# tkeskita/smoothMesh

Measured on AMD Instinct MI355X. Metric: mesh-points smoothed/sec/node (100 iters) + achieved HBM GB/s vs roofline, higher is better.
Workload: dtype f64

## Files before the change

### smoothmesh_amd/csrc/kernels_tiled.hpp

```cpp
#pragma once
#include "kernels.hpp"
#include "tile_meta.hpp"

#ifndef SMGPU_STAGGER
#define SMGPU_STAGGER 0
#endif
__device__ __forceinline__ void staggerFirstRound(int bid, int resident) {
#if SMGPU_STAGGER
    if (bid < resident) {
        const unsigned slot = __builtin_amdgcn_s_getreg((3 << 11) | (0 << 6) | 4) & 15u;
        for (unsigned k = 0; k < slot; ++k) __builtin_amdgcn_s_sleep(SMGPU_STAGGER);
    }
#else
    (void)bid; (void)resident;
#endif
}
#ifndef SMGPU_ABLATE
#define SMGPU_ABLATE 0
#endif
namespace smgpu {

constexpr unsigned kPad = 0xFFFFu;

struct GeomTileView {
// ... 447 lines not shown
    if (tm.nPts > 2 * T)
        stageRecords<T, 2, kGP>(s.ptsCur, g.tpIds + tm.tpOff + 2 * T, tm.nPts - 2 * T, L.px + kGP * 2 * T, L.py + kGP * 2 * T, L.pz + kGP * 2 * T, tid);
}
template <int T, bool ORG>
__device__ __forceinline__ void geomFaces(const State& s, const GeomTileView& g, const GeomLds& L, const GeomTileMeta& tm, const GeomRows& r, int tid,
                                          int wantAvg, int writeFaces) {
    const unsigned tflags = (unsigned)tm.flags;
    const int nf = tm.nFaces;
#pragma unroll
    for (int u = 0; u < 2; ++u) {
        const int i = u * T + tid;
        if (i < nf) geomFace<ORG>(s, g, L, tm, i, tflags, wantAvg, writeFaces, r.preFaces, r.fq[u]);
    }
    for (int i = 2 * T + tid; i < nf; i += T) geomFace<ORG>(s, g, L, tm, i, tflags, wantAvg, writeFaces);
}

template <int T, bool ORG>
__device__ __forceinline__ void geomTileBody(const TileLaunch& tl, const MeshView& m, const State& s, const GeomTileView& g, int wantAvg, int writeFaces,
                                             int deferN, int deferIter, double* deferLocal, double* deferHist, int bid, bool coh = false) {
    const int tile = launchedTile(tl, bid);
    if (tile < 0) return;
    const GeomTileMeta tm = loadGeomMeta(tl.meta, tile);
    const int stopped = stopWord(tl);
    scalarBatch(tm.tpOff, tm.nPts, tm.tfOff, tm.nFaces, tm.fvBase, tm.fvWidth, tm.cellBeg, tm.nCells, tm.cfBase, tm.cfWidth, tm.flags, stopped,
                g.tpIds, g.faceVerts, g.cellOrder, g.cellFaces, s.ptsCur, deferN);
    staggerFirstRound(bid, 256 * 4);
    if (deferN > 0 && bid == 0) { if (stopped) return; finishPartials<T>(s, deferN, deferIter, -1.0, deferLocal, deferHist); __syncthreads(); }
    extern __shared__ double lds[];
    const int tid = threadIdx.x;
    const GeomLds L = geomLds(lds, tm);
    int id[2];
    geomLoadIds<T>(g, tm, tid, id);
    const GeomRows r = geomLoadRows<T, ORG>(g, tm, tid);
    V3 v[2];
    geomLoadPoints(s, id, v);
    geomStorePoints<T>(s, g, tm, L, id, v, tid);
    if (stopped) return;
    prologuePrioDown<1>();
    __syncthreads();
    if (SMGPU_ABLATE & 32) { if (tid < tm.nCells) stv(s.cellCtr, ((const_int_ptr)g.cellOrder)[tm.cellBeg + tid], v3(L.px[tid], 0.0, 0.0)); return; }
    geomFaces<T, ORG>(s, g, L, tm, r, tid, wantAvg, writeFaces);
    __syncthreads();
    if (SMGPU_ABLATE & 64) return;
    geomCell<T, ORG>(s, g, L, tm, tid, (unsigned)tm.flags, r.cin, coh);
}
template <int T, bool ORG>
__global__ void __launch_bounds__(T, (SMGPU_GEOM_WAVES * T) / 256) k_geom_tile(TileLaunch tl, MeshView m, State s, GeomTileView g, int wantAvg, int writeFaces,
                                                  int deferN, int deferIter, double* deferLocal, double* deferHist) {
    prologuePrioUp<1>();
    geomTileBody<T, ORG>(tl, m, s, g, wantAvg, writeFaces, deferN, deferIter, deferLocal, deferHist, (int)blockIdx.x);
}

struct SmoothLds { double *cx, *cy, *cz, *nx, *ny, *nz; };
__device__ __forceinline__ SmoothLds smoothLds(double* lds, const SmoothTileMeta& tm) {
    SmoothLds L;
    L.cx = lds;                 L.cy = L.cx + tm.nCells;  L.cz = L.cy + tm.nCells;
    L.nx = L.cz + tm.nCells;    L.ny = L.nx + tm.nNbrs;   L.nz = L.ny + tm.nNbrs;
    return L;
}
struct Top3 {
    double l1 = 0, l2 = 0, l3 = 0;
    unsigned w1 = 0xFFFFFFFFu, w2 = 0xFFFFFFFFu, w3 = 0xFFFFFFFFu;
    __device__ __forceinline__ void offer(double len, int j, unsigned e, bool take) {
        const unsigned w = ((unsigned)j << 16) | e;
        const bool b1 = take && (w1 == 0xFFFFFFFFu || len < l1);
        const bool b2 = take && !b1 && (w2 == 0xFFFFFFFFu || len < l2);
        const bool b3 = take && !b1 && !b2 && (w3 == 0xFFFFFFFFu || len < l3);
        const bool b12 = b1 || b2;
        l3 = b12 ? l2 : (b3 ? len : l3);  w3 = b12 ? w2 : (b3 ? w : w3);
        l2 = b1 ? l1 : (b2 ? len : l2);   w2 = b1 ? w1 : (b2 ? w : w2);
        l1 = b1 ? len : l1;               w1 = b1 ? w : w1;
    }
    __device__ __forceinline__ bool has2() const { return w2 != 0xFFFFFFFFu; }
    __device__ __forceinline__ bool has3() const { return w3 != 0xFFFFFFFFu; }
    __device__ __forceinline__ int k1() const { return (int)(w1 >> 16); }
    __device__ __forceinline__ int k2() const { return (int)(w2 >> 16); }
};
struct SmoothRow {
    bool mine; int p, selfL, wn4, wc4, slot;
    int peer, dst0, ndst;
    unsigned fl;
    const ushort4 *ppRow, *pcRow;
    ushort4 pp0, pp1, pc0, pc1;
    ushort4 pe0, pe1;
};
template <int T>
__device__ __forceinline__ unsigned pairBits(const SmoothTileView& g, const SmoothTileMeta& tm, const SmoothRow& R, int tid, int k) {
    if (k < 8) {
        const ushort4 q = (k & 4) ? R.pe1 : R.pe0;
        const unsigned lo = (k & 1) ? q.y : q.x, hi = (k & 1) ? q.w : q.z;
        return (k & 2) ? hi : lo;
    }
    const uint16_t* pe = g.pairEll + tm.ppBase;
    return pe[((size_t)(k >> 2) * T + tid) * 4 + (k & 3)];
}
struct SlotTabs { const int* slot; const int* peer; const int* dst0; const int* ndst; };
template <int T, bool COHC = false, int SLOTS = 1>
__device__ __forceinline__ SmoothRow smoothStage(const MeshView& m, const State& s, const SmoothTileView& g, const SmoothTileMeta& tm,
                                                 const SmoothLds& L, int tid, const SlotTabs& tb = SlotTabs{nullptr, nullptr, nullptr, nullptr}) {
    scalarBatch(tm.ptBeg, tm.nPts, tm.tcOff, tm.nCells, tm.tnOff, tm.nNbrs, tm.pcBase, tm.pcWidth, tm.ppBase, tm.ppWidth,
                g.tcIds, g.tnIds, g.ptOrder, g.selfLoc, g.ppEll, g.pcEll, g.pairEll, g.usePairShare, s.cellCtr, s.ptsCur, m.pflags);
    if (SLOTS == 1) scalarBatch(s.sharedSlot);
    if (SLOTS == 2) scalarBatch(tb.slot, tb.peer, tb.dst0, tb.ndst);
    SmoothRow r;
    r.peer = -1; r.dst0 = -1; r.ndst = 0;
    r.mine = tid < tm.nPts;
    r.wn4 = tm.ppWidth >> 2; r.wc4 = tm.pcWidth >> 2;
    const int lane = r.mine ? tid : 0;
    r.ppRow = reinterpret_cast<const ushort4*>(g.ppEll + tm.ppBase) + tid;
    r.pcRow = reinterpret_cast<const ushort4*>(g.pcEll + tm.pcBase) + tid;
    const bool fast = tm.nCells <= 2 * T && tm.nNbrs <= 3 * T && r.wn4 > 0 && r.wc4 > 0;
    const ushort4 padq = make_ushort4(0xFFFF, 0xFFFF, 0xFFFF, 0xFFFF);
    if (fast) {
        const int* ic = g.tcIds + tm.tcOff;
        const int* in = g.tnIds + tm.tnOff;
        int a[2], b[3];
#pragma unroll
        for (int u = 0; u < 2; ++u) { const int i = u * T + tid; a[u] = (i < tm.nCells) ? ic[i] : -1; }
#pragma unroll
        for (int u = 0; u < 3; ++u) { const int i = u * T + tid; b[u] = (i < tm.nNbrs) ? in[i] : -1; }
        const int pi = tm.ptBeg + lane;
        const int p = g.ptOrder[pi];
        const int selfL = g.selfLoc[pi];
        const ushort4* ppl = reinterpret_cast<const ushort4*>(g.ppEll + tm.ppBase) + lane;
        const ushort4* pcl = reinterpret_cast<const ushort4*>(g.pcEll + tm.pcBase) + lane;
        const ushort4 pp0 = ppl[0], pp1 = ppl[r.wn4 > 1 ? T : 0], pc0 = pcl[0], pc1 = pcl[r.wc4 > 1 ? T : 0];
        const ushort4* pel = reinterpret_cast<const ushort4*>((g.usePairShare ? g.pairEll : g.ppEll) + tm.ppBase) + lane;
        r.pe0 = pel[0]; r.pe1 = pel[r.wn4 > 1 ? T : 0];
        int slot = -1, peer = -1, dst0 = -1, ndst = 0;
        if (SLOTS == 2) { slot = tb.slot[pi]; if (tb.peer) { peer = tb.peer[pi]; dst0 = tb.dst0[pi]; ndst = tb.ndst[pi]; } }
        V3 va[2], vb[3];
#pragma unroll
        for (int u = 0; u < 2; ++u) va[u] = (a[u] >= 0) ? (COHC ? ldvCoh(s.cellCtr, a[u]) : ldv(s.cellCtr, a[u])) : v3(0, 0, 0);
#pragma unroll
        for (int u = 0; u < 3; ++u) vb[u] = (b[u] >= 0) ? ldv(s.ptsCur, b[u]) : v3(0, 0, 0);
        const unsigned fl = m.pflags[p];
        if (SLOTS == 1) slot = s.sharedSlot ? s.sharedSlot[p] : -1;
#pragma unroll
        for (int u = 0; u < 2; ++u) { const int i = u * T + tid; if (a[u] >= 0) { L.cx[i] = va[u].x; L.cy[i] = va[u].y; L.cz[i] = va[u].z; } }
#pragma unroll
        for (int u = 0; u < 3; ++u) { const int i = u * T + tid; if (b[u] >= 0) { L.nx[i] = vb[u].x; L.ny[i] = vb[u].y; L.nz[i] = vb[u].z; } }
        r.p = r.mine ? p : 0; r.selfL = r.mine ? selfL : 0;
        r.fl = fl; r.slot = r.mine ? slot : -1; r.peer = r.mine ? peer : -1; r.dst0 = dst0; r.ndst = r.mine ? ndst : 0;
        r.pp0 = r.mine ? pp0 : padq; r.pp1 = (r.mine && r.wn4 > 1) ? pp1 : padq;
        r.pc0 = r.mine ? pc0 : padq; r.pc1 = (r.mine && r.wc4 > 1) ? pc1 : padq;
        return r;
    }
    r.p = 0; r.selfL = 0; r.fl = 0; r.slot = -1;
    r.pp0 = padq; r.pp1 = padq; r.pc0 = padq; r.pc1 = padq; r.pe0 = padq; r.pe1 = padq;
    if (r.mine) {
        if (g.usePairShare) {
            const ushort4* peRow = reinterpret_cast<const ushort4*>(g.pairEll + tm.ppBase) + tid;
            if (r.wn4 > 0) r.pe0 = peRow[0];
            if (r.wn4 > 1) r.pe1 = peRow[T];
        }
        const int pi = tm.ptBeg + tid;
        r.p = g.ptOrder[pi];
        r.selfL = g.selfLoc[pi];
        if (r.wn4 > 0) r.pp0 = r.ppRow[0];
        if (r.wn4 > 1) r.pp1 = r.ppRow[T];
        if (r.wc4 > 0) r.pc0 = r.pcRow[0];
        if (r.wc4 > 1) r.pc1 = r.pcRow[T];
        r.fl = m.pflags[r.p];
        if (SLOTS == 1) r.slot = s.sharedSlot ? s.sharedSlot[r.p] : -1;
        if (SLOTS == 2) { r.slot = tb.slot[pi]; if (tb.peer) { r.peer = tb.peer[pi]; r.dst0 = tb.dst0[pi]; r.ndst = tb.ndst[pi]; } }
    }
    if (COHC) stageRecordsCoh<T>(s.cellCtr, g.tcIds + tm.tcOff, tm.nCells, L.cx, L.cy, L.cz, tid);
    else stageRecords<T, 2>(s.cellCtr, g.tcIds + tm.tcOff, tm.nCells, L.cx, L.cy, L.cz, tid);
    stageRecords<T, 3>(s.ptsCur, g.tnIds + tm.tnOff, tm.nNbrs, L.nx, L.ny, L.nz, tid);
    return r;
}

template <bool FINAL, int T, int MODE = 0>
__device__ __forceinline__ void smoothPoint(const MeshView& m, const State& s, const Prm& prm, const SmoothTileView& g, const SmoothLds& L,
                                            const SmoothRow& R, const SmoothTileMeta& tm, int tid, double& dist, int& fcount, bool spTile = false) {
    const double *cx = L.cx, *cy = L.cy, *cz = L.cz, *nx = L.nx, *ny = L.ny, *nz = L.nz;
    const bool mine = R.mine;
    const int p = R.p, selfL = R.selfL, wn4 = R.wn4, wc4 = R.wc4;
    const ushort4 *ppRow = R.ppRow, *pcRow = R.pcRow;
    const ushort4 pp0 = R.pp0, pp1 = R.pp1, pc0 = R.pc0, pc1 = R.pc1;
    if ((SMGPU_ABLATE & 16) && !spTile) { if (mine) stv(FINAL ? s.ptsNext : s.prop, p, ldsv(nx, ny, nz, selfL)); return; }
    if (mine && !(MODE == 2 && !spTile && R.slot >= 0)) {
        const unsigned fl = R.fl;
        const bool internal = fl & PF_INTERNAL;
        const V3 cur = ldsv(nx, ny, nz, selfL);
        V3 sum = v3(0, 0, 0), r1, r2, r3;
        double m1 = 0.0, m2 = 0.0, m3 = 0.0;
        int count = 0, hc = 0;
        double shortestCur = SMGPU_GREAT;
        const int slot = (MODE == 1 || (MODE == 2 && !spTile)) ? -1 : R.slot;
        if (slot >= 0) {
            {
                const double* r = s.combA + (size_t)slot * SMGPU_HALO_A_DOUBLES;
                double w[SMGPU_HALO_A_DOUBLES];
#pragma unroll
                for (int q = 0; q < SMGPU_HALO_A_DOUBLES; ++q) w[q] = (MODE == 2 && R.peer < 0) ? ldCoh(r + q) : r[q];
                sum = v3(w[0], w[1], w[2]);
                r1 = v3(w[3], w[4], w[5]); r2 = v3(w[6], w[7], w[8]); r3 = v3(w[9], w[10], w[11]);
                const long long pk = __double_as_longlong(w[12]);
                count = (int)(pk & 0xffffffffll);
                hc = (int)(pk >> 32);
            }
            m1 = mag(r1); m2 = mag(r2); m3 = mag(r3);
            SMGPU_ELL_FOREACH_PRE(pp0, pp1, ppRow, wn4, T, {
                (void)j;
                const double len = mag(cur - ldsv(nx, ny, nz, e & 0x7fff));
                if (len < shortestCur) shortestCur = len;
            })
        } else {
            if (internal || prm.bndOn) {
                if (!(SMGPU_ABLATE & 8))
                SMGPU_ELL_FOREACH_PRE(pc0, pc1, pcRow, wc4, T, {
                    sum = sum + ldsv(cx, cy, cz, (SMGPU_ABLATE & 2) ? 0 : e);
                    count = j + 1;
                })
            }
            Top3 t3;
            SMGPU_ELL_FOREACH_PRE(pp0, pp1, ppRow, wn4, T, {
                const V3 dv_ = cur - ldsv(nx, ny, nz, (SMGPU_ABLATE & 2) ? 0 : (e & 0x7fff));
                const double len = (SMGPU_ABLATE & 1) ? magSqr(dv_) : mag(dv_);
                if (len < shortestCur) shortestCur = len;
                t3.offer(len, j, e, internal || !(e & 0x8000));
            })
            if (!t3.has2()) { s.acc->err = 1; r1 = r2 = r3 = v3(0, 0, 0); }
            else {
                r1 = ldsv(nx, ny, nz, t3.w1 & 0x7fff) - cur;
                r2 = ldsv(nx, ny, nz, t3.w2 & 0x7fff) - cur;
                r3 = !t3.has3() ? v3(SMGPU_GREAT, SMGPU_GREAT, SMGPU_GREAT) : ldsv(nx, ny, nz, t3.w3 & 0x7fff) - cur;
                m1 = t3.l1; m2 = t3.l2; m3 = !t3.has3() ? mag(r3) : t3.l3;
                if (g.usePairShare) {
                    hc = (pairBits<T>(g, tm, R, tid, t3.k1()) >> t3.k2()) & 1;
                } else {
                    const int nb = m.ppOff[p];
                    hc = shareCell(m, m.ppPt[nb + t3.k1()], m.ppPt[nb + t3.k2()]) ? 1 : 0;
                }
            }
        }
        V3 np = cur;
        if (count) np = divByCount(sum, count);
        const double blendFrac = arRatioLen(r1, r2, m1, m2, m3, hc != 0, internal);
        if (blendFrac > 0.0) {
            const V3 aCoords = cur + 0.5 * (r1 + r2);
            np = (1.0 - blendFrac) * np + blendFrac * aCoords;
        }
        {
            const V3 stepDir = np - cur;
            const double len = mag(stepDir);
            const double globalScale = (len > prm.maxStep) ? prm.maxStep / (len * prm.relStepFrac) : 1.0;
            np = cur + (prm.relStepFrac * globalScale) * stepDir;
        }
        if (prm.layersOn) np = layerTreat(s, prm, p, internal, cur, np);
        const bool deferBnd = prm.bndOn && !internal;
        if (prm.bndOn && internal) {
            const V3 stepDir = np - cur;
            const double len = mag(stepDir);
            const double globalScale = (len > prm.maxStep) ? prm.maxStep / (len * prm.relStepFrac) : 1.0;
            np = cur + (prm.relStepFrac * globalScale) * stepDir;
        }
        bool frozen = false;
        {
            double minSqr = __builtin_inf();
            if (!(SMGPU_ABLATE & 4))
            SMGPU_ELL_FOREACH_PRE(pp0, pp1, ppRow, wn4, T, {
                (void)j;
                const double t2 = magSqr(np - ldsv(nx, ny, nz, (SMGPU_ABLATE & 2) ? 0 : (e & 0x7fff)));
                if (t2 < minSqr) minSqr = t2;
            })
            const double rootMin = sqrtExact(minSqr);
            const double shortestNew = (rootMin < SMGPU_GREAT) ? rootMin : SMGPU_GREAT;
            const double shortest = (shortestNew < shortestCur) ? shortestNew : shortestCur;
            if (prm.totalMinFreeze && (shortest < prm.minEdge)) frozen = true;
            else if ((shortestNew < prm.minEdge) && (shortestNew < shortestCur)) frozen = true;
        }
        if (deferBnd) stv(s.prop, p, np);
        else if (FINAL && slot >= 0) {
            if (MODE == 2 && s.ownF) {
                stvCoh(s.prop, p, np);
                __hip_atomic_store(s.ownF + slot, frozen ? 1 : 0, __ATOMIC_RELAXED, __HIP_MEMORY_SCOPE_AGENT);
            } else stv(s.prop, p, np);
            s.frozen[p] = frozen ? 1 : 0;
            if (MODE == 2) {
                const int v = frozen ? 1 : 0;
                if (R.ndst == 1) { if (s.push.slotF) stPeer(s.push.slotF[R.dst0], v); else s.sendF[R.dst0] = v; }
                else
                    for (int k = s.sendOff[slot]; k < s.sendOff[slot + 1]; ++k) {
                        const int sl = s.sendSlots[k];
                        if (s.push.slotF) stPeer(s.push.slotF[sl], v); else s.sendF[sl] = v;
                    }
            } else if (s.inlinePackF)
                for (int k = s.sendOff[slot]; k < s.sendOff[slot + 1]; ++k) s.sendF[s.sendSlots[k]] = frozen ? 1 : 0;
        } else if (FINAL) {
            if (frozen || (!internal && !(fl & PF_SMOOTHSURF))) { np = cur; fcount = 1; }
            dist = mag(np - cur) / prm.maxStep;
            stv(s.ptsNext, p, np);
        } else {
            stv(s.prop, p, np);
            s.frozen[p] = frozen ? 1 : 0;
            if (s.stepSqr) s.stepSqr[p] = magSqr(np - cur);
        }
    }
}

template <bool FINAL, int T>
__global__ void __launch_bounds__(T) k_smooth_tile(TileLaunch tl, MeshView m, State s, Prm prm, SmoothTileView g) {
    prologuePrioUp<2>();
    const int tile = launchedTile(tl, (int)blockIdx.x);
    if (tile < 0) return;
    const SmoothTileMeta tm = loadSmoothMeta(tl.meta, tile);
    const int stopped = stopWord(tl);
    scalarBatch(stopped);
    staggerFirstRound((int)blockIdx.x, 256 * 6);
    extern __shared__ double lds[];
    const int tid = threadIdx.x;
    const SmoothLds L = smoothLds(lds, tm);
    const SmoothRow R = smoothStage<T>(m, s, g, tm, L, tid);
    if (stopped) return;
    prologuePrioDown<2>();
    __syncthreads();
    double dist = 0.0;
    int fcount = 0;
    smoothPoint<FINAL, T>(m, s, prm, g, L, R, tm, tid, dist, fcount);
    if (FINAL) blockPublish<T>(s, dist, fcount, tile);
}

struct PackView {
    double* ownA; double* sendA;
    const int* sendOff; const int* sendSlots;
    int centroidAll;
};
template <int T, bool COHC = false, bool SP = false>
__device__ __forceinline__ void packTileBody(const TileLaunch& tl, const MeshView& m, const State& s, const SmoothTileView& g, const PackView& pk, int bid) {
    const int tile = launchedTile(tl, bid);
    if (tile < 0) return;
    extern __shared__ double lds[];
    const int tid = threadIdx.x;
    const SmoothTileMeta tm = loadSmoothMeta(tl.meta, tile);
    const SmoothLds L = smoothLds(lds, tm);
    const SmoothRow R = smoothStage<T, COHC, SP ? 2 : 1>(m, s, g, tm, L, tid, SlotTabs{s.spSlot, s.spPeer, s.spDst0, s.spNDst});
    __syncthreads();
    if (!R.mine) return;
    const int p = R.p;
    const int slot = R.slot;
    if (slot < 0) return;
    const double *cx = L.cx, *cy = L.cy, *cz = L.cz, *nx = L.nx, *ny = L.ny, *nz = L.nz;
    const int wn4 = R.wn4, wc4 = R.wc4;
    const ushort4 *ppRow = R.ppRow, *pcRow = R.pcRow;
    const ushort4 pp0 = R.pp0, pp1 = R.pp1, pc0 = R.pc0, pc1 = R.pc1;
    const bool internal = R.fl & PF_INTERNAL;
    const V3 cur = ldsv(nx, ny, nz, R.selfL);
    V3 sum = v3(0, 0, 0), r1, r2, r3;
    int count = 0, hc = 0;
    if (internal || pk.centroidAll) {
        SMGPU_ELL_FOREACH_PRE(pc0, pc1, pcRow, wc4, T, {
            sum = sum + ldsv(cx, cy, cz, e);
            count = j + 1;
        })
    }
    Top3 t3;
    SMGPU_ELL_FOREACH_PRE(pp0, pp1, ppRow, wn4, T, {
        const double len = mag(cur - ldsv(nx, ny, nz, e & 0x7fff));
        t3.offer(len, j, e, internal || !(e & 0x8000));
    })
    if (!t3.has2()) { s.acc->err = 1; r1 = r2 = r3 = v3(0, 0, 0); }
    else {
        r1 = ldsv(nx, ny, nz, t3.w1 & 0x7fff) - cur;
        r2 = ldsv(nx, ny, nz, t3.w2 & 0x7fff) - cur;
        r3 = !t3.has3() ? v3(SMGPU_GREAT, SMGPU_GREAT, SMGPU_GREAT) : ldsv(nx, ny, nz, t3.w3 & 0x7fff) - cur;
        if (g.usePairShare) {
            hc = (pairBits<T>(g, tm, R, tid, t3.k1()) >> t3.k2()) & 1;
        } else {
            const int nb = m.ppOff[p];
            hc = shareCell(m, m.ppPt[nb + t3.k1()], m.ppPt[nb + t3.k2()]) ? 1 : 0;
        }
    }
    double rec[SMGPU_HALO_A_DOUBLES];
// ... 159 lines not shown
```

### smoothmesh_amd/csrc/setup_create.hpp

```cpp
#pragma once

struct SetupTasks {
    std::vector<int32_t> pointOrder;
    std::future<std::vector<int32_t>> fPointOrder;
    std::future<TileTables> geom, smooth, edge;
    CornerChains chains;
    DeviceTopologyArrays owned;
    void fetchPointOrder() { if (fPointOrder.valid()) pointOrder = fPointOrder.get(); }
    void join() {
        if (fPointOrder.valid()) fPointOrder.wait();
        for (std::future<TileTables>* f : {&geom, &smooth, &edge}) if (f->valid()) f->wait();
    }
    ~SetupTasks() { join(); releaseCornerChains(chains); releaseOwned(owned); }
};
static int startTasksAndAddressing(smgpu_handle* h, const smgpu_mesh_desc* d, SetupTasks& tasks) {
    const TilePlan& plan = h->plan;
    const DeviceTopologyArrays& lists = h->devLists;
    h->gt.latticeKeys = h->stl.latticeKeys = h->etl.latticeKeys = plan.latticeKeys;
    if (plan.wantTiles && plan.morton) tasks.fPointOrder = std::async(std::launch::async, [d, &plan] { return mortonOrderOf(d->nPoints, d->points, plan.latticeKeys); });
    const std::vector<int32_t>* po = &tasks.pointOrder;
    const auto afterCells = [&] {
        if (!plan.wantTiles || !plan.shapesOk()) return;
        if (plan.deviceTiles == 1 && lists.valid) {
            std::string why;
// ... 34 lines not shown
            [h, d, &plan, po] {
                return h->etl.buildBoundaries(h->topo, d->points, plan.morton, 256, plan.capEdgePoints, plan.capEdgeFaces, plan.capEdgeCells, (plan.morton && !po->empty()) ? po : nullptr,
                                              plan.capEdgeTotal);
            },
            [h, &lists](std::string& why) { return buildEdgeTablesOnDevice(h->etl, lists, h->topo.nEdges, h->device, h->etDev, why); },
            [h] { return h->etl.buildTables(h->topo); });
    };
    int dev = envInt("SMGPU_DEVICE_TOPOLOGY", 1) ? 1 : -1;
    if (dev > 0) {
        std::string why;
        dev = buildTopologyOnDevice(h->topo, d->nPoints, d->nCells, d->nFaces, d->nInternalFaces, d->faceOffsets, d->facePoints, d->owner, d->neighbour, h->device, why,
                                    afterCells, afterPoints, &h->devLists, startEdge, plan.deviceTiles != 0 && plan.wantTiles);
        tasks.owned = h->devLists;
        if (dev == 2) return fail("smgpu_create: device addressing: " + why);
        if (plan.verbose >= 1) std::fprintf(stderr, "[smgpu] addressing on the %s (%.2f s since create)\n", dev == 0 ? "device" : "host (device path handed the mesh back)", setupClock());
    }
    if (dev != 0) {
        h->topo = Topology();
        const std::string terr = h->topo.build(d->nPoints, d->nCells, d->nFaces, d->nInternalFaces, d->faceOffsets, d->facePoints, d->owner, d->neighbour, afterCells, afterPoints);
        if (!terr.empty()) return fail("smgpu_create: " + terr);
    }
    startEdge();
    return 0;
}

static int installAddressing(smgpu_handle* h, const smgpu_mesh_desc* d, SetupTasks& tasks) {
    const Topology& t = h->topo;
    MeshView& m = h->mv;
    m.nPoints = t.nPoints; m.nCells = t.nCells; m.nFaces = t.nFaces; m.nInternalFaces = t.nInternalFaces; m.nEdges = t.nEdges;
    std::vector<uint8_t> flags(t.nPoints);
    for (int p = 0; p < t.nPoints; ++p)
        flags[p] = (d->isInternalPoint[p] ? PF_INTERNAL : 0) |
                   ((d->isSmoothingSurfacePoint && d->isSmoothingSurfacePoint[p]) ? PF_SMOOTHSURF : 0);
    int rc = 0;
    const bool onDev = tasks.owned.valid;
#define SMGPU_X(name, list) rc |= place(h, onDev, m.name, tasks.owned.name, t.list);
    SMGPU_ADDRESSING(SMGPU_X)
#undef SMGPU_X
    rc |= devUpload(h, &m.pflags, flags);
    return rc;
}

static void readLoopKnobs(smgpu_handle* h) {
    h->useTiles = h->plan.wantTiles;
    h->useFilter = h->plan.wantFilter;
    h->xcdMap = envInt("SMGPU_XCD_MAP", 1) != 0;
    h->walkStar = envInt("SMGPU_WALK_STAR", 1) != 0;
    h->starBlocks = std::max(1, envInt("SMGPU_STAR_BLOCKS", 256 * 32));
    h->walkPack = envInt("SMGPU_WALK_PACK", 1) != 0;
    h->walkCache = envInt("SMGPU_WALK_CACHE", 1) != 0;
    h->faLists = envInt("SMGPU_FA_LISTS", 1) != 0;
    h->faSideExact = envInt("SMGPU_FA_SIDE_EXACT", 1) != 0;
    h->bndInGeom = envInt("SMGPU_BND_IN_GEOM", 1) != 0;
    h->qt.fusedWanted = envInt("SMGPU_QUALITY_TRACE_FUSED", 1) != 0;
    { const char* fv = std::getenv("SMGPU_FOAM_VARIANT"); h->foamOrg = fv && std::string(fv) == "org"; }
    { const char* sv = std::getenv("SMGPU_SYNC_VARIANT"); h->st.ownFold = (sv && std::string(sv) == "own") ? 1 : 0; }
}

static int installTiles(smgpu_handle* h, SetupTasks& tasks, double tTopo, const std::function<void(const char*)>& lap) {
    const TilePlan& plan = h->plan;
    h->geomT = plan.geomT;
    h->smoothT = plan.smoothT;
    if (!TilePlan::shapeOk(plan.geomT)) return fail("SMGPU_GEOM_T must be 64, 128 or 256");
    if (!TilePlan::shapeOk(plan.smoothT)) return fail("SMGPU_SMOOTH_T must be 64, 128 or 256");
    tasks.join();
    auto fetched = [&](int groups) { std::string why; return downloadDeferredLists(h->topo, h->devLists, h->device, why, groups) == 0; };
    const bool geomOk = tileTablesStand(tasks.geom, [&] { return h->gt.buildTables(h->topo); });
    const bool smoothOk = tileTablesStand(tasks.smooth, [&] { return fetched(1) ? h->stl.buildTables(h->topo, h->isInternalHost.data()) : std::string("no lists"); });
    const bool edgeOk = tileTablesStand(tasks.edge, [&] { return fetched(2) ? h->etl.buildTables(h->topo) : std::string("no lists"); });
    if (plan.verbose) std::fprintf(stderr, "[smgpu] set-up: addressing %.2f s, tile tables (3 host threads) %.2f s\n", tTopo, setupClock() - tTopo);
    releaseOwned(tasks.owned);
    lap("tile tasks joined");
    if (!geomOk || !smoothOk) { h->useTiles = false; return 0; }
    if (installGeomTiles(h)) return 1;
    if (installSmoothTiles(h, h->stl, h->stDev, h->sv, h->topo.maxPointPoints <= 16 ? 1 : 0, true)) return 1;
    if (h->useFilter && edgeOk && installEdgeTiles(h)) return 1;
    {
        size_t mx = 0;
        for (int ti = 0; ti < h->gt.nTiles; ++ti)
            mx = std::max(mx, 3 * (size_t)(h->gt.tpOff[(size_t)ti + 1] - h->gt.tpOff[(size_t)ti]) +
                                  (size_t)(SMGPU_GEOM_AOS ? kGF : 6) * (size_t)(h->gt.tfOff[(size_t)ti + 1] - h->gt.tfOff[(size_t)ti]));
        h->geomLds = sizeof(double) * mx;
    }
    h->smoothLds = sizeof(double) * 3 * maxTileTotal(h->stl.nTiles, {&h->stl.tcOff, &h->stl.tnOff});
    if (plan.verbose)
        std::fprintf(stderr, "[smgpu] tiles: geom T=%d n=%d LDS=%zu B (maxP %d maxF %d; staged faces x%.3f, points x%.3f of the mesh's)  smooth T=%d n=%d LDS=%zu B (maxC %d maxN %d)\n",
                     h->geomT, h->gt.nTiles, h->geomLds, h->gv.maxPoints, h->gv.maxFaces, (double)h->gt.tfOff.back() / std::max(1, h->topo.nFaces),
                     (double)h->gt.tpOff.back() / std::max(1, h->topo.nPoints), h->smoothT, h->stl.nTiles, h->smoothLds, h->sv.maxCells, h->sv.maxPoints);
    return 0;
}

static void sizeEdgeAngle(smgpu_handle* h) {
    const Topology& t = h->topo;
    const char* ea = std::getenv("SMGPU_EDGE_ANGLE");
    h->eaCoop = !(ea && std::string(ea) == "faithful");
    for (int p0 = 0; p0 < t.nPoints; p0 += kEaPointsPerBlock) {
        const int p1 = std::min(t.nPoints, p0 + kEaPointsPerBlock);
        h->eaMaxEntries = std::max(h->eaMaxEntries, t.pointEdges.off[p1] - t.pointEdges.off[p0]);
    }
    if (sizeof(double) * 9 * (size_t)h->eaMaxEntries > 60 * 1024) h->eaCoop = false;
}

static int allocWorkArrays(smgpu_handle* h) {
    const Topology& t = h->topo;
    State& s = h->st;
    const size_t P = t.nPoints, C = t.nCells, F = t.nFaces, E = t.nEdges;
    int rc = 0;
    rc |= devAlloc(h, &h->bufA, 3 * P);
    rc |= devAlloc(h, &h->bufB, 3 * P);
    rc |= devAlloc(h, &s.prop, 3 * P);
    rc |= devAlloc(h, &h->dStepSqr, P + 4);
    rc |= devAlloc(h, &s.fCtr, 3 * F);
    rc |= devAlloc(h, &s.fArea, 3 * F);
    s.avgPacked = (h->useTiles && h->edgeTilesOk && h->avgPackedCount) ? 1 : 0;
    rc |= devAlloc(h, &s.fAvg, 3 * (s.avgPacked ? h->avgPackedCount : F));
    rc |= devAlloc(h, &s.cellCtr, 3 * C);
    rc |= devAlloc(h, &s.frozen, P);
    rc |= devAlloc(h, &s.edgeMin, E);
    rc |= devAlloc(h, &s.edgeMax, E);
    rc |= devAlloc(h, &s.ptMin, P);
    rc |= devAlloc(h, &s.ptMax, P);
    rc |= devAlloc(h, &s.faActive, P + 16);
    rc |= devAlloc(h, &h->dFaMaybe, P + 16);
    rc |= devAlloc(h, &s.faEdgeList, E);
    rc |= devAlloc(h, &s.faPointList, P);
    rc |= devAlloc(h, &h->dEaMaybe, P);
    rc |= devAlloc(h, &s.faS, P);
    rc |= devAlloc(h, &s.faN, t.pointPoints.size());
    rc |= devAlloc(h, &s.walkStack, P + 64);
    rc |= devAlloc(h, &s.acc, 1);
    rc |= devAlloc(h, &s.nearTotal, 4);
    const size_t nPart = (size_t)std::max(gridFor(t.nPoints), h->useTiles ? h->stl.nTiles : 0) + 2 * (size_t)gridFor(t.nPoints) + 1;
    rc |= devAlloc(h, &s.blkMax, nPart);
    rc |= devAlloc(h, &s.blkCnt, nPart);
    return rc;
}

static int uploadPoints(smgpu_handle* h, const smgpu_mesh_desc* d) {
    State& s = h->st;
    const size_t P = (size_t)h->topo.nPoints;
    if (hipMemset(s.acc, 0, sizeof(Accum)) != hipSuccess) return fail("hipMemset failed");
// ... 26 lines not shown
```

### smoothmesh_amd/csrc/smgpu.hip

```cpp
#include <hip/hip_runtime.h>
#include <hip/hip_ext.h>

#include <algorithm>
#include <chrono>
#include <future>
#include <memory>
#include <mutex>
#include <cstdio>
#include <cstring>
#include <string>
#include <vector>

#include "kernels.hpp"
#include "layers.hpp"
#include "kernels_tiled.hpp"
#include "kernels_walk.hpp"
#include "kernels_filter.hpp"
#include "kernels_boundary.hpp"
#include "kernels_quality.hpp"
#include "kernels_quality_geom.hpp"
#include "kernels_quality_motion.hpp"
#include "kernels_quality_trace.hpp"
#include "kernels_quality_guard.hpp"
#include "kernels_quality_tangle.hpp"
// ... 62 lines not shown
    std::vector<uint8_t> sharedMasterHost;
    std::unique_ptr<LayerBuilder> lb;
    std::vector<double> lbArea;
    std::vector<uint8_t> lbInternal;
    int *sendF = nullptr, *recvF = nullptr;
    double* localStats = nullptr;
    double* statsHistory = nullptr;
    int32_t statsHistoryCap = 0;
    int64_t statsHistoryN = 0;
    int haloIter = 0;
    bool pushOn = false;
    int pushPeers = 0, pushStride = 0;
    std::vector<int32_t> pushCount, pushRemoteBase, pushMyIndex;
    std::vector<void*> pushRecvA, pushRecvL, pushRecvF, pushFlags;
    void* pushLocalFlags = nullptr;
    unsigned long long pushTimeoutTicks = 6000000000ull;
    void *dSlotA = nullptr, *dSlotL = nullptr, *dSlotF = nullptr, *dPeerFlag = nullptr;
    unsigned* dPushTicket = nullptr;
    int *dInteriorTiles = nullptr, *dSharedTiles = nullptr;
    int nInteriorTiles = 0, nSharedTiles = 0;
    bool interiorDone = false;
    int *dGeomInterior = nullptr, *dGeomShared = nullptr;
    int nGeomInterior = 0, nGeomShared = 0;
    bool geomAheadDone = false;
    int* dPosSlot = nullptr;
    SmoothTiles shr;
    SmoothTileView hv{};
    size_t haloLds = 0;
    std::vector<uint8_t> isInternalHost;
    unsigned* dRoleTickets = nullptr;
    unsigned roleLaunches[3] = {0, 0, 0};
    int* dOwnF = nullptr;
    bool fixInSmooth = false;
    bool mergedWanted = true;
    bool flagWanted = true;
    bool flagBuilt = false;
    uint32_t* dFlagWords = nullptr;
    void *dSelfSlotA = nullptr, *dSelfSlotF = nullptr, *dSelfPeerFlag = nullptr;
    unsigned* dSelfTicket = nullptr;
    PushView flagView{};
    bool mergedIter = false;
    TilePlan plan;
    bool useTiles = false;
    int geomT = 128, smoothT = 256;
    GeomTiles gt;
    GeomTilesDev gtDev;
    EdgeTilesDev etDev;
    SmoothTilesDev stDev;
    DeviceTopologyArrays devLists;
    SmoothTiles stl;
    GeomTileView gv{};
    SmoothTileView sv{};
    size_t geomLds = 0, smoothLds = 0;
    bool writeFaces = false;
    int walkMode = -1;
    bool walkForced = false;
    int walkSwitches = 0;
    int* nActiveHost = nullptr;
    long walkDecisions = 0;
    hipEvent_t evWalkLag[2] = {nullptr, nullptr};
    unsigned long long* dWalkOps = nullptr;
    unsigned long long* dWalkMemo = nullptr;
    unsigned long long walkMemoLast[2] = {0, 0};
    bool walkAlloc = false;
    WalkView wv{};
    FixView fxw{};
    bool fixAlloc = false;
    int walkFixBlocks = 128;
    int deviceShare = 1;
    double* dStepSqr = nullptr;
    int walkSweeps = 8;
    bool bndInGeom = true;
    bool bndPreDone = false;
    bool faSideExact = true;
    bool faExactOnSide = false;
    bool walkPack = true;
    bool walkCache = true;
    StarCache starCache{nullptr, nullptr, nullptr, 0};
    int starBlocks = 256 * 32;
    bool faLists = true;
    bool walkStar = true;
    int walkBlocks = 0;
    void* pinned = nullptr;
    size_t pinnedBytes = 0;
    std::vector<uint8_t> walkFrozen;
    std::vector<int> walkStack, walkOut;
    std::vector<char> walkHost;
    bool useFilter = true, exactAll = false;
    uint8_t *dFaMaybe = nullptr, *dEaMaybe = nullptr;
    bool eaFilterRan = false, faFilterRan = false;
    hipStream_t side = nullptr;
    hipEvent_t evFork = nullptr, evJoin = nullptr;
    uint32_t* depWords = nullptr;
    uint32_t depValue[8] = {0, 0, 0, 0, 0, 0, 0, 0};
    bool streamOps = false;
    int deferN = 0, deferIter = 0;
    double* deferLocal = nullptr;
    double* deferHist = nullptr;
    bool foamOrg = false;
    int xcdMap = 1;
    bool layersOn = false;
    bool packTiles = true;
    bool bndOn = false;
    hipStream_t bndSide = nullptr;
    hipEvent_t evBndFork = nullptr, evBndJoin = nullptr;
    bool bndPreInFlight = false;
// ... 398 lines not shown
int smgpu_set_foam_variant(smgpu_handle* h, int32_t variant) {
    if (!h) return fail("null handle");
    if (variant != SMGPU_FOAM_COM && variant != SMGPU_FOAM_ORG) return fail("smgpu_set_foam_variant: unknown variant");
    h->foamOrg = variant == SMGPU_FOAM_ORG;
    h->q.epoch++;
    h->geomAheadDone = false;
    return 0;
}

int smgpu_set_sync_variant(smgpu_handle* h, int32_t variant) {
    if (!h) return fail("null handle");
    if (variant != SMGPU_SYNC_MASTER && variant != SMGPU_SYNC_OWN) return fail("smgpu_set_sync_variant: unknown variant");
    h->st.ownFold = variant == SMGPU_SYNC_OWN ? 1 : 0;
    return 0;
}

int smgpu_set_params(smgpu_handle* h, const smgpu_params* p) {
    if (!h || !p) return fail("null argument");
    if (!(p->maxStepLength > 0.0)) return fail("maxStepLength must be > 0");
    h->prm = *p;
    h->prmSet = true;
    h->walkMode = -1;
    h->walkSwitches = 0;
    h->walkDecisions = 0;
    if (h->nActiveHost) *(volatile int*)h->nActiveHost = -1;
    h->geomAheadDone = false;
    computeAlgoBytes(h);
    return 0;
}

extern "C++" {
template <typename K>
static void ensureDynLds(K kernel, int device, size_t bytes) {
    static std::mutex mu;
    static size_t have[64] = {0};
    if (bytes <= 64 * 1024 || device < 0 || device >= 64) return;
    std::lock_guard<std::mutex> lock(mu);
    if (have[device] >= bytes) return;
    if (hipFuncSetAttribute((const void*)kernel, hipFuncAttributeMaxDynamicSharedMemorySize, (int)bytes) == hipSuccess) have[device] = bytes;
    else (void)hipGetLastError();
}
template <class F>
static void withGeomTile(const smgpu_handle* h, F&& f) {
    auto variant = [&](auto t) {
        if (h->foamOrg) f(t, std::true_type{});
        else f(t, std::false_type{});
    };
    if (h->geomT == 64) variant(std::integral_constant<int, 64>{});
    else if (h->geomT == 128) variant(std::integral_constant<int, 128>{});
    else variant(std::integral_constant<int, 256>{});
}
template <bool FINAL, int T>
static void launchSmoothTile(smgpu_handle* h, const MeshView& m, const State& s, const Prm& prm, const int* tileList, int nTiles, hipEvent_t evA, hipEvent_t evB) {
    ensureDynLds(k_smooth_tile<FINAL, T>, h->device, h->smoothLds);
    hipExtLaunchKernelGGL((k_smooth_tile<FINAL, T>), dim3(tileGrid(nTiles, h->xcdMap)), dim3(T), (uint32_t)h->smoothLds, h->stream, evA, evB, 0,
                          tileLaunch(h->sv.meta, s, tileList, nTiles, h->xcdMap), m, s, prm, h->sv);
}
template <bool FINAL>
static int launchBndFix(smgpu_handle* h, int partialBase) {
    if (h->bv.nB == 0) return 0;
    return launchK(h, K_BND, [&] {
        hipLaunchKernelGGL(k_bnd_fix<FINAL>, dim3(gridFor(2 * (int64_t)h->bv.nB)), dim3(kBlock), 0, h->stream, h->mv, h->st, makePrm(h), h->bv, partialBase);
    });
}
static int launchBndPre(smgpu_handle* h, const MeshView& m, const State& s, hipStream_t stream) {
    if (h->bv.nB == 0) return 0;
    return launchK(h, K_BND, [&] {
        hipLaunchKernelGGL(k_bnd_normals, dim3(gridFor(h->bv.nB)), dim3(kBlock), 0, stream, m, s, h->bv);
        if (h->bv.nFeat) hipLaunchKernelGGL(k_bnd_feature, dim3(h->bv.nFeat), dim3(64), 0, stream, m, s, h->bv);
    }, stream);
}
static int runBndPre(smgpu_handle* h) {
    if (h->bndOn && h->bndInGeom && h->useTiles && h->bv.nB > 0) return 0;
    if (!h->bndOn || !h->bndSide || h->bndPreInFlight || h->timing) return 0;
    if (depSignal(h, DEP_BND_FORK, h->stream, h->evBndFork) || depWait(h, DEP_BND_FORK, h->bndSide, h->evBndFork)) return 1;
    if (launchBndPre(h, h->mv, h->st, h->bndSide)) return 1;
    if (depSignal(h, DEP_BND_JOIN, h->bndSide, h->evBndJoin)) return 1;
    h->bndPreInFlight = true;
    return 0;
}
template <bool FINAL>
static int runSmooth(smgpu_handle* h, const MeshView& m, const State& s, const Prm& prm, const int* tileList = nullptr, int nList = 0) {
    const int kid = FINAL ? K_SMOOTH_FINAL : K_SMOOTH_PROP;
    const bool withBnd = h->bndOn && !h->haloOn;
    if (withBnd) {
        if (h->bndPreDone) h->bndPreDone = false;
        else if (h->bndPreInFlight) {
            if (depWait(h, DEP_BND_JOIN, h->stream, h->evBndJoin)) return 1;
            h->bndPreInFlight = false;
        } else if (launchBndPre(h, m, s, h->stream)) return 1;
    }
    if (h->useTiles) {
        const int nT = tileList ? nList : h->stl.nTiles;
        if (nT == 0) return 0;
        if (launchKDispatch(h, kid, [&](hipEvent_t evA, hipEvent_t evB) {
                if (h->smoothT == 64) launchSmoothTile<FINAL, 64>(h, m, s, prm, tileList, nT, evA, evB);
                else if (h->smoothT == 128) launchSmoothTile<FINAL, 128>(h, m, s, prm, tileList, nT, evA, evB);
                else launchSmoothTile<FINAL, 256>(h, m, s, prm, tileList, nT, evA, evB);
            })) return 1;
    } else if (launchK(h, kid, [&] { hipLaunchKernelGGL(k_smooth<FINAL>, dim3(gridFor(m.nPoints)), dim3(kBlock), 0, h->stream, m, s, prm); })) return 1;
    if (withBnd) {
        const int base = h->useTiles ? h->stl.nTiles : gridFor(m.nPoints);
        return launchK(h, K_BND, [&] { hipLaunchKernelGGL(k_bnd_fix<FINAL>, dim3(gridFor(2 * (int64_t)h->bv.nB)), dim3(kBlock), 0, h->stream, m, s, prm, h->bv, base); });
    }
    return 0;
}

}

// ... 2026 lines not shown
```

Before: 13.00 billion.

## Overlay smooth-tile LDS regions by precomputing centroid sums before staging neighbors

The smooth tile kernel now computes each point's cell-centroid sum and count right after staging cell centres into LDS. It then reuses the same LDS region for the neighbour points, so the dynamic LDS becomes the max rather than the sum of the two regions. A SOLO variant without shared-slot handling is selected when halo exchange is off, and some kernel arguments (State, Prm, MeshView) are re-read late from the kernarg segment to shorten register live ranges. The aim is higher occupancy. The cost is two extra block barriers per tile and more template variants.

```diff
diff --git a/smoothmesh_amd/csrc/kernels_tiled.hpp b/smoothmesh_amd/csrc/kernels_tiled.hpp
--- a/smoothmesh_amd/csrc/kernels_tiled.hpp
+++ b/smoothmesh_amd/csrc/kernels_tiled.hpp
@@ -523,10 +523,11 @@
 }
 
 struct SmoothLds { double *cx, *cy, *cz, *nx, *ny, *nz; };
+template <bool OVL = false>
 __device__ __forceinline__ SmoothLds smoothLds(double* lds, const SmoothTileMeta& tm) {
     SmoothLds L;
-    L.cx = lds;                 L.cy = L.cx + tm.nCells;  L.cz = L.cy + tm.nCells;
-    L.nx = L.cz + tm.nCells;    L.ny = L.nx + tm.nNbrs;   L.nz = L.ny + tm.nNbrs;
+    L.cx = lds;                          L.cy = L.cx + tm.nCells;  L.cz = L.cy + tm.nCells;
+    L.nx = OVL ? lds : L.cz + tm.nCells; L.ny = L.nx + tm.nNbrs;   L.nz = L.ny + tm.nNbrs;
     return L;
 }
 struct Top3 {
@@ -554,7 +555,21 @@
     const ushort4 *ppRow, *pcRow;
     ushort4 pp0, pp1, pc0, pc1;
     ushort4 pe0, pe1;
+    V3 sum; int count;
 };
+template <int T>
+__device__ __forceinline__ void smoothCentroid(const SmoothLds& L, SmoothRow& r, int centroidAll) {
+    V3 sum = v3(0, 0, 0);
+    int count = 0;
+    if (r.mine && r.slot < 0 && ((r.fl & PF_INTERNAL) || centroidAll)) {
+        if (!(SMGPU_ABLATE & 8))
+        SMGPU_ELL_FOREACH_PRE(r.pc0, r.pc1, r.pcRow, r.wc4, T, {
+            sum = sum + ldsv(L.cx, L.cy, L.cz, (SMGPU_ABLATE & 2) ? 0 : e);
+            count = j + 1;
+        })
+    }
+    r.sum = sum; r.count = count;
+}
 template <int T>
 __device__ __forceinline__ unsigned pairBits(const SmoothTileView& g, const SmoothTileMeta& tm, const SmoothRow& R, int tid, int k) {
     if (k < 8) {
@@ -566,15 +581,18 @@
     return pe[((size_t)(k >> 2) * T + tid) * 4 + (k & 3)];
 }
 struct SlotTabs { const int* slot; const int* peer; const int* dst0; const int* ndst; };
-template <int T, bool COHC = false, int SLOTS = 1>
+template <int T, bool COHC = false, int SLOTS = 1, bool OVL = false>
 __device__ __forceinline__ SmoothRow smoothStage(const MeshView& m, const State& s, const SmoothTileView& g, const SmoothTileMeta& tm,
-                                                 const SmoothLds& L, int tid, const SlotTabs& tb = SlotTabs{nullptr, nullptr, nullptr, nullptr}) {
+                                                 const SmoothLds& L, int tid, const SlotTabs& tb = SlotTabs{nullptr, nullptr, nullptr, nullptr},
+                                                 int centroidAll = 0) {
     scalarBatch(tm.ptBeg, tm.nPts, tm.tcOff, tm.nCells, tm.tnOff, tm.nNbrs, tm.pcBase, tm.pcWidth, tm.ppBase, tm.ppWidth,
                 g.tcIds, g.tnIds, g.ptOrder, g.selfLoc, g.ppEll, g.pcEll, g.pairEll, g.usePairShare, s.cellCtr, s.ptsCur, m.pflags);
     if (SLOTS == 1) scalarBatch(s.sharedSlot);
     if (SLOTS == 2) scalarBatch(tb.slot, tb.peer, tb.dst0, tb.ndst);
+    if (OVL) scalarBatch(centroidAll);
     SmoothRow r;
     r.peer = -1; r.dst0 = -1; r.ndst = 0;
+    r.sum = v3(0, 0, 0); r.count = 0;
     r.mine = tid < tm.nPts;
     r.wn4 = tm.ppWidth >> 2; r.wc4 = tm.pcWidth >> 2;
     const int lane = r.mine ? tid : 0;
@@ -609,12 +627,17 @@
         if (SLOTS == 1) slot = s.sharedSlot ? s.sharedSlot[p] : -1;
 #pragma unroll
         for (int u = 0; u < 2; ++u) { const int i = u * T + tid; if (a[u] >= 0) { L.cx[i] = va[u].x; L.cy[i] = va[u].y; L.cz[i] = va[u].z; } }
-#pragma unroll
-        for (int u = 0; u < 3; ++u) { const int i = u * T + tid; if (b[u] >= 0) { L.nx[i] = vb[u].x; L.ny[i] = vb[u].y; L.nz[i] = vb[u].z; } }
         r.p = r.mine ? p : 0; r.selfL = r.mine ? selfL : 0;
         r.fl = fl; r.slot = r.mine ? slot : -1; r.peer = r.mine ? peer : -1; r.dst0 = dst0; r.ndst = r.mine ? ndst : 0;
         r.pp0 = r.mine ? pp0 : padq; r.pp1 = (r.mine && r.wn4 > 1) ? pp1 : padq;
         r.pc0 = r.mine ? pc0 : padq; r.pc1 = (r.mine && r.wc4 > 1) ? pc1 : padq;
+        if (OVL) {
+            __syncthreads();
+            smoothCentroid<T>(L, r, centroidAll);
+            __syncthreads();
+        }
+#pragma unroll
+        for (int u = 0; u < 3; ++u) { const int i = u * T + tid; if (b[u] >= 0) { L.nx[i] = vb[u].x; L.ny[i] = vb[u].y; L.nz[i] = vb[u].z; } }
         return r;
     }
     r.p = 0; r.selfL = 0; r.fl = 0; r.slot = -1;
@@ -638,11 +661,30 @@
     }
     if (COHC) stageRecordsCoh<T>(s.cellCtr, g.tcIds + tm.tcOff, tm.nCells, L.cx, L.cy, L.cz, tid);
     else stageRecords<T, 2>(s.cellCtr, g.tcIds + tm.tcOff, tm.nCells, L.cx, L.cy, L.cz, tid);
+    if (OVL) {
+        __syncthreads();
+        smoothCentroid<T>(L, r, centroidAll);
+        __syncthreads();
+    }
     stageRecords<T, 3>(s.ptsCur, g.tnIds + tm.tnOff, tm.nNbrs, L.nx, L.ny, L.nz, tid);
     return r;
 }
 
-template <bool FINAL, int T, int MODE = 0>
+typedef const __attribute__((address_space(4))) char* const_arg_ptr;
+template <class A>
+__device__ __forceinline__ A lateArg(size_t off) {
+    const_arg_ptr p = (const_arg_ptr)__builtin_amdgcn_kernarg_segment_ptr();
+    asm volatile("" : "+s"(p));
+    A a;
+    __builtin_memcpy(&a, reinterpret_cast<const __attribute__((address_space(4))) A*>(p + off), sizeof(A));
+    return a;
+}
+constexpr size_t argOffset(size_t end, size_t align) { return (end + align - 1) / align * align; }
+constexpr size_t kSmoothArgM = argOffset(sizeof(TileLaunch), alignof(MeshView));
+constexpr size_t kSmoothArgS = argOffset(kSmoothArgM + sizeof(MeshView), alignof(State));
+constexpr size_t kSmoothArgP = argOffset(kSmoothArgS + sizeof(State), alignof(Prm));
+
+template <bool FINAL, int T, int MODE = 0, bool OVL = false, bool LATE = false>
 __device__ __forceinline__ void smoothPoint(const MeshView& m, const State& s, const Prm& prm, const SmoothTileView& g, const SmoothLds& L,
                                             const SmoothRow& R, const SmoothTileMeta& tm, int tid, double& dist, int& fcount, bool spTile = false) {
     const double *cx = L.cx, *cy = L.cy, *cz = L.cz, *nx = L.nx, *ny = L.ny, *nz = L.nz;
@@ -679,7 +721,8 @@
                 if (len < shortestCur) shortestCur = len;
             })
         } else {
-            if (internal || prm.bndOn) {
+            if (OVL) { sum = R.sum; count = R.count; }
+            else if (internal || prm.bndOn) {
                 if (!(SMGPU_ABLATE & 8))
                 SMGPU_ELL_FOREACH_PRE(pc0, pc1, pcRow, wc4, T, {
                     sum = sum + ldsv(cx, cy, cz, (SMGPU_ABLATE & 2) ? 0 : e);
@@ -701,6 +744,10 @@
                 m1 = t3.l1; m2 = t3.l2; m3 = !t3.has3() ? mag(r3) : t3.l3;
                 if (g.usePairShare) {
                     hc = (pairBits<T>(g, tm, R, tid, t3.k1()) >> t3.k2()) & 1;
+                } else if (LATE) {
+                    const MeshView ml = lateArg<MeshView>(kSmoothArgM);
+                    const int nb = ml.ppOff[p];
+                    hc = shareCell(ml, ml.ppPt[nb + t3.k1()], ml.ppPt[nb + t3.k2()]) ? 1 : 0;
                 } else {
                     const int nb = m.ppOff[p];
                     hc = shareCell(m, m.ppPt[nb + t3.k1()], m.ppPt[nb + t3.k2()]) ? 1 : 0;
@@ -720,7 +767,10 @@
             const double globalScale = (len > prm.maxStep) ? prm.maxStep / (len * prm.relStepFrac) : 1.0;
             np = cur + (prm.relStepFrac * globalScale) * stepDir;
         }
-        if (prm.layersOn) np = layerTreat(s, prm, p, internal, cur, np);
+        if (prm.layersOn) {
+            if (LATE) { const State sl = lateArg<State>(kSmoothArgS); np = layerTreat(sl, prm, p, internal, cur, np); }
+            else np = layerTreat(s, prm, p, internal, cur, np);
+        }
         const bool deferBnd = prm.bndOn && !internal;
         if (prm.bndOn && internal) {
             const V3 stepDir = np - cur;
@@ -772,7 +822,7 @@
     }
 }
 
-template <bool FINAL, int T>
+template <bool FINAL, int T, bool SOLO = false, bool OVL = false>
 __global__ void __launch_bounds__(T) k_smooth_tile(TileLaunch tl, MeshView m, State s, Prm prm, SmoothTileView g) {
     prologuePrioUp<2>();
     const int tile = launchedTile(tl, (int)blockIdx.x);
@@ -783,15 +833,17 @@
     staggerFirstRound((int)blockIdx.x, 256 * 6);
     extern __shared__ double lds[];
     const int tid = threadIdx.x;
-    const SmoothLds L = smoothLds(lds, tm);
-    const SmoothRow R = smoothStage<T>(m, s, g, tm, L, tid);
+    const SmoothLds L = smoothLds<OVL>(lds, tm);
+    const SmoothRow R = smoothStage<T, false, SOLO ? 0 : 1, OVL>(m, s, g, tm, L, tid, SlotTabs{nullptr, nullptr, nullptr, nullptr}, prm.bndOn);
     if (stopped) return;
     prologuePrioDown<2>();
     __syncthreads();
     double dist = 0.0;
     int fcount = 0;
-    smoothPoint<FINAL, T>(m, s, prm, g, L, R, tm, tid, dist, fcount);
-    if (FINAL) blockPublish<T>(s, dist, fcount, tile);
+    const State sL = lateArg<State>(kSmoothArgS);
+    const Prm prmL = lateArg<Prm>(kSmoothArgP);
+    smoothPoint<FINAL, T, SOLO ? 1 : 0, OVL, true>(m, sL, prmL, g, L, R, tm, tid, dist, fcount);
+    if (FINAL) blockPublish<T>(sL, dist, fcount, tile);
 }
 
 struct PackView {
diff --git a/smoothmesh_amd/csrc/setup_create.hpp b/smoothmesh_amd/csrc/setup_create.hpp
--- a/smoothmesh_amd/csrc/setup_create.hpp
+++ b/smoothmesh_amd/csrc/setup_create.hpp
@@ -110,6 +110,7 @@
     h->faLists = envInt("SMGPU_FA_LISTS", 1) != 0;
     h->faSideExact = envInt("SMGPU_FA_SIDE_EXACT", 1) != 0;
     h->bndInGeom = envInt("SMGPU_BND_IN_GEOM", 1) != 0;
+    h->smoothOverlay = envInt("SMGPU_SMOOTH_OVERLAY", 1) != 0;
     h->qt.fusedWanted = envInt("SMGPU_QUALITY_TRACE_FUSED", 1) != 0;
     { const char* fv = std::getenv("SMGPU_FOAM_VARIANT"); h->foamOrg = fv && std::string(fv) == "org"; }
     { const char* sv = std::getenv("SMGPU_SYNC_VARIANT"); h->st.ownFold = (sv && std::string(sv) == "own") ? 1 : 0; }
@@ -141,10 +142,13 @@
         h->geomLds = sizeof(double) * mx;
     }
     h->smoothLds = sizeof(double) * 3 * maxTileTotal(h->stl.nTiles, {&h->stl.tcOff, &h->stl.tnOff});
+    h->smoothLdsOvl = sizeof(double) * 3 * std::max(maxTileTotal(h->stl.nTiles, {&h->stl.tcOff}), maxTileTotal(h->stl.nTiles, {&h->stl.tnOff}));
     if (plan.verbose)
-        std::fprintf(stderr, "[smgpu] tiles: geom T=%d n=%d LDS=%zu B (maxP %d maxF %d; staged faces x%.3f, points x%.3f of the mesh's)  smooth T=%d n=%d LDS=%zu B (maxC %d maxN %d)\n",
+        std::fprintf(stderr, "[smgpu] tiles: geom T=%d n=%d LDS=%zu B (maxP %d maxF %d; staged faces x%.3f, points x%.3f of the mesh's)  smooth T=%d n=%d LDS=%zu B (maxC %d maxN %d)"
+                             "  smooth overlay %s LDS=%zu B\n",
                      h->geomT, h->gt.nTiles, h->geomLds, h->gv.maxPoints, h->gv.maxFaces, (double)h->gt.tfOff.back() / std::max(1, h->topo.nFaces),
-                     (double)h->gt.tpOff.back() / std::max(1, h->topo.nPoints), h->smoothT, h->stl.nTiles, h->smoothLds, h->sv.maxCells, h->sv.maxPoints);
+                     (double)h->gt.tpOff.back() / std::max(1, h->topo.nPoints), h->smoothT, h->stl.nTiles, h->smoothLds, h->sv.maxCells, h->sv.maxPoints,
+                     h->smoothOverlay ? "on" : "off", h->smoothOverlay ? h->smoothLdsOvl : h->smoothLds);
     return 0;
 }
 
diff --git a/smoothmesh_amd/csrc/smgpu.hip b/smoothmesh_amd/csrc/smgpu.hip
--- a/smoothmesh_amd/csrc/smgpu.hip
+++ b/smoothmesh_amd/csrc/smgpu.hip
@@ -138,6 +138,8 @@
     GeomTileView gv{};
     SmoothTileView sv{};
     size_t geomLds = 0, smoothLds = 0;
+    size_t smoothLdsOvl = 0;
+    bool smoothOverlay = true;
     bool writeFaces = false;
     int walkMode = -1;
     bool walkForced = false;
@@ -642,9 +644,16 @@
 }
 template <bool FINAL, int T>
 static void launchSmoothTile(smgpu_handle* h, const MeshView& m, const State& s, const Prm& prm, const int* tileList, int nTiles, hipEvent_t evA, hipEvent_t evB) {
-    ensureDynLds(k_smooth_tile<FINAL, T>, h->device, h->smoothLds);
-    hipExtLaunchKernelGGL((k_smooth_tile<FINAL, T>), dim3(tileGrid(nTiles, h->xcdMap)), dim3(T), (uint32_t)h->smoothLds, h->stream, evA, evB, 0,
-                          tileLaunch(h->sv.meta, s, tileList, nTiles, h->xcdMap), m, s, prm, h->sv);
+    auto go = [&](auto solo, auto ovl) {
+        constexpr bool SOLO = decltype(solo)::value, OVL = decltype(ovl)::value;
+        const size_t lds = OVL ? h->smoothLdsOvl : h->smoothLds;
+        ensureDynLds(k_smooth_tile<FINAL, T, SOLO, OVL>, h->device, lds);
+        hipExtLaunchKernelGGL((k_smooth_tile<FINAL, T, SOLO, OVL>), dim3(tileGrid(nTiles, h->xcdMap)), dim3(T), (uint32_t)lds, h->stream, evA, evB, 0,
+                              tileLaunch(h->sv.meta, s, tileList, nTiles, h->xcdMap), m, s, prm, h->sv);
+    };
+    const bool solo = !h->haloOn && !s.sharedSlot;
+    if (solo) { if (h->smoothOverlay) go(std::true_type{}, std::true_type{}); else go(std::true_type{}, std::false_type{}); }
+    else { if (h->smoothOverlay) go(std::false_type{}, std::true_type{}); else go(std::false_type{}, std::false_type{}); }
 }
 template <bool FINAL>
 static int launchBndFix(smgpu_handle* h, int partialBase) {
```

Result: no change. 13.13 billion, median of 6 (+1.0%).
